# chalkydri/chalkydri

Measured on AMD Instinct MI355X. Metric: frames/sec (detect+pose) on 1280x800 batch; HBM GB/s vs roofline, higher is better.
Workload: dtype u8 (threshold/segment/clusters: integer; quad fit/decode/SQPnP: f64)

## Files before the change

chalkydri_amd/csrc/ck_internal.h:

```cpp
#ifndef CK_INTERNAL_H
#define CK_INTERNAL_H

#include <hip/hip_runtime.h>
#include <stdint.h>
#include <stdio.h>
#include <stdlib.h>

#include "chalkydri_hip.h"

typedef uint16_t ck_label_t;
#define CK_LBL_BORDER 0x8000u
#define CK_LBL_SMALL 0x4000u
#define CK_LBL_LOCAL_MASK 0x0FFFu
#define CK_LBL_ID_MASK 0x01FFu
#define CK_LBL_NONE 0xFFFFu
#define CK_LBL_INVALID 0xFFFFFFFFu

#define CK_TW 128
#define CK_TH 32
#define CK_RING_CAP (2 * (CK_TW + CK_TH))

__host__ __device__ inline uint32_t ck_label_slot(uint32_t l, int x, int y, int ccl_tiles_x) {
    return (uint32_t)((y / CK_TH) * ccl_tiles_x + x / CK_TW) * (uint32_t)CK_RING_CAP + (l & CK_LBL_ID_MASK);
}
__host__ __device__ inline uint32_t ck_label_interior_root(uint32_t l, int x, int y, int w) {
    return (uint32_t)((y & ~(CK_TH - 1)) + (int)((l >> 7) & (CK_TH - 1))) * (uint32_t)w + (uint32_t)((x & ~(CK_TW - 1)) + (int)(l & (CK_TW - 1)));
}

struct ck_border_root {
    uint32_t root;
    uint32_t size;
};

struct ck_dev_family {
    uint32_t nbits, ncodes, n_upstream;
    int32_t width_at_border, total_width, reversed_border;
    const uint64_t *codes;
    uint32_t bit_x[64], bit_y[64];
};

constexpr int CK_FIT_CLASSES = 8;
constexpr int CK_FIT_LISTS = 9;
constexpr int CK_EXT_PRE = 25, CK_EXT_POST = 24, CK_EXT_HALO = CK_EXT_PRE + CK_EXT_POST;
constexpr int CK_SPAN = 960;
constexpr int CK_HUGE_CAP = 65536, CK_HUGE_WGS = 256;
constexpr int CK_FIT_PARALLEL_MAX_FRAMES = 16;
constexpr int CK_SEG_CHUNKS_MAX = 8;
constexpr int CK_FIT_SIDE_STREAMS = 2;
constexpr int CK_LSCRATCH_PER_WG = 16384, CK_LSCRATCH_WGS = 1024;

typedef uint32_t ck_packed_point;
__host__ __device__ inline ck_cluster_point_t ck_unpack_point(ck_packed_point v) {
    const int k = (int)(v >> 1) & 3, sgn = (v & 1u) ? 1 : -1;
    const int dx = k == 2 ? -1 : (k == 1 ? 0 : 1), dy = k == 0 ? 0 : 1;
    ck_cluster_point_t p;
    p.x = (uint16_t)((v >> 16) & 0x1FFFu); p.y = (uint16_t)((v >> 3) & 0x1FFFu);
    p.gx = (int8_t)(dx * sgn); p.gy = (int8_t)(dy * sgn); p.pad = 0;
    return p;
}
struct ck_run {
    uint32_t slot;
    uint32_t base;
    uint32_t tmp_start;
    uint32_t count;
};

struct ck_stage_ws {
    int ht_size;
    int point_cap, cluster_cap, quad_cap, det_cap;
    int max_cluster_points;
    unsigned long long *d_ht_keys;
    uint32_t *d_ht_count;
    uint32_t *d_ht_off;
    ck_packed_point *d_tmp;
    ck_packed_point *d_points;
    int ext_cap;
    uint32_t *d_ext_xy;
    uint16_t *d_ext_w;
    double *d_maxval;
    uint16_t *d_maxpos;
    unsigned long long *d_maxmask;
    uint16_t *d_maxpre;
    long long *d_blk;
    uint32_t *d_cstate;
    ck_run *d_runs;
    int run_cap;
    unsigned long long *d_lscratch;
    unsigned long long *d_hscratch;
    int hcap;
    ck_cluster_t *d_clusters;
    uint32_t *d_counters;
    ck_quad_t *d_quads;
    ck_detection_t *d_dets;
    uint16_t *d_wimg;
    void *d_fit_scratch;
    size_t fit_scratch_bytes;
    ck_field_tag_t *d_field; int field_cap;
    double *d_gyro; uint8_t *d_has_gyro;
    ck_sqpnp_problem_t *d_problems;
    ck_iso3_t *d_pose_tags;
    double *d_bearings;
    double *d_world;
    ck_sqpnp_result_t *d_results;
    ck_vision_measurement_t *d_meas;
    int32_t *d_valid;
};
#define CK_CNT_TMP 0
#define CK_CNT_CLUSTERS 1
#define CK_CNT_POINTS 2
#define CK_CNT_QUADS 3
#define CK_CNT_DETS 4
#define CK_CNT_STATUS 5
#define CK_CNT_RUNS 6
#define CK_CNT_EXT 7
#define CK_CNT_STRIDE 8

struct ck_handle {
    ck_config_t cfg;
    int device;
    hipStream_t stream;
    hipStream_t stream2;
    hipEvent_t ev[16];
    hipEvent_t ev_fork, ev_join;
    hipStream_t fit_stream[CK_FIT_SIDE_STREAMS];
    hipStream_t seg_stream;
// ... 174 lines not shown
```

chalkydri_amd/csrc/k_quads.hip:

```cpp
#include <stdlib.h>

#include "ck_internal.h"

namespace {

struct FitArgs {
    const uint8_t *qim; int qw, qh, qstride; size_t qpitch;
    const uint16_t *wimg;
    const uint8_t *im; int w, h, stride; size_t pitch;
    int decimate, refine, max_nmaxima, min_tag_width, normal_ok, reversed_ok;
    double cos_critical, max_mse;
    ck_stage_ws ws;
    int stop_after;
    int guided;
    int list_cap;
    const uint32_t *list;
    const uint32_t *list_count;
    uint32_t *head;
};

struct M6 { long long Mx, My, Mxx, Mxy, Myy, W; };
__device__ __forceinline__ M6 m6_add(M6 a, M6 b) { a.Mx += b.Mx; a.My += b.My; a.Mxx += b.Mxx; a.Mxy += b.Mxy; a.Myy += b.Myy; a.W += b.W; return a; }
__device__ __forceinline__ M6 m6_sub(M6 a, M6 b) { a.Mx -= b.Mx; a.My -= b.My; a.Mxx -= b.Mxx; a.Mxy -= b.Mxy; a.Myy -= b.Myy; a.W -= b.W; return a; }
__device__ __forceinline__ M6 m6_zero() { M6 z = {0, 0, 0, 0, 0, 0}; return z; }
// ... 1231 lines not shown
#pragma unroll
                for (int e = 0; e < EPL; e++) {
                    const int i = tid + e * NTH;
                    if (i < sz0) {
                        const unsigned long long raw = stage(rawp[e]);
                        sKeys[i] = raw;
                        const int px = (int)(raw & 0xFFFF), py = (int)((raw >> 16) & 0xFFFF);
                        xmin = min(xmin, px); xmax = max(xmax, px);
                        ymin = min(ymin, py); ymax = max(ymax, py);
                    }
                }
            } else {
                for (int i = tid; i < sz0; i += NTH) {
                    const unsigned long long raw = stage(pts[i]);
                    sKeys[i] = raw;
                    const int px = (int)(raw & 0xFFFF), py = (int)((raw >> 16) & 0xFFFF);
                    xmin = min(xmin, px); xmax = max(xmax, px);
                    ymin = min(ymin, py); ymax = max(ymax, py);
                }
            }
            {
                int bb[4] = {xmin, -xmax, ymin, -ymax};
                B::reduce_min4(bb, iscr);
                xmin = bb[0]; xmax = -bb[1]; ymin = bb[2]; ymax = -bb[3];
            }
            if ((xmax - xmin) * (ymax - ymin) < a.min_tag_width) continue;
            if (a.stop_after == 10) continue;
            long long dot;
            {
                constexpr int EPLS = CAP / NTH;
                int n2 = NTH;
                while (n2 < sz0) n2 <<= 1;
                const int epl = n2 / NTH;
                B::sync();
                bool sorted = false;
                if constexpr (MLDS)
                    dot = keys_bucket_sort<NTH, EPLS>(sKeys, reinterpret_cast<uint32_t *>(sHist), sScratch, sz0, xmin, xmax, ymin, ymax,
                                                      a.normal_ok, a.reversed_ok, a.stop_after != 11, &sorted);
                else
                    dot = keys_bucket_sort_global<NTH, GK>(sKeys, reinterpret_cast<uint32_t *>(sHist), sScratch, scratch8, sz0, xmin, xmax, ymin, ymax,
                                                           a.normal_ok, a.reversed_ok, a.stop_after != 11, &sorted);
                if (sorted || GK) {}
                else if (EPLS >= 32 && epl == 32) dot = keys_sort<NTH, (EPLS >= 32 && !GK ? 32 : 1)>(sKeys, sScratch, sz0, xmin, xmax, ymin, ymax, a.normal_ok, a.reversed_ok, a.stop_after != 11);
                else if (EPLS >= 16 && epl == 16) dot = keys_sort<NTH, (EPLS >= 16 && !GK ? 16 : 1)>(sKeys, sScratch, sz0, xmin, xmax, ymin, ymax, a.normal_ok, a.reversed_ok, a.stop_after != 11);
                else if (EPLS >= 8 && epl == 8) dot = keys_sort<NTH, (EPLS >= 8 && !GK ? 8 : 1)>(sKeys, sScratch, sz0, xmin, xmax, ymin, ymax, a.normal_ok, a.reversed_ok, a.stop_after != 11);
                else if (EPLS >= 4 && epl == 4) dot = keys_sort<NTH, (EPLS >= 4 && !GK ? 4 : 1)>(sKeys, sScratch, sz0, xmin, xmax, ymin, ymax, a.normal_ok, a.reversed_ok, a.stop_after != 11);
                else if (EPLS >= 2 && epl == 2) dot = keys_sort<NTH, (EPLS >= 2 && !GK ? 2 : 1)>(sKeys, sScratch, sz0, xmin, xmax, ymin, ymax, a.normal_ok, a.reversed_ok, a.stop_after != 11);
                else dot = keys_sort<NTH, 1>(sKeys, sScratch, sz0, xmin, xmax, ymin, ymax, a.normal_ok, a.reversed_ok, a.stop_after != 11);
            }
            const int reversed = dot < 0;
            if (reversed && !a.reversed_ok) continue;
            if (!reversed && !a.normal_ok) continue;
            if (a.stop_after == 1 || a.stop_after == 11) continue;
            B::sync();
            int sz = 0;
            for (int base = 0; base < sz0; base += NTH) {
                const int i = base + tid;
                unsigned long long key = 0;
                int keep = 0;
                if (i < sz0) { key = sKeys[i]; keep = (i == 0) || (sKeys[i - 1] != key); }
                int tot = 0;
                const int incl = B::scan_flag(keep, iscr, &tot);
                B::sync();
                if (keep) sXY[sz + (int)incl - 1] = (uint32_t)(key & 0x3FFFFFFu);
                sz += (int)tot;
                B::sync();
            }
            if (sz < 24) continue;
            const int ksz = sz / 12 < 20 ? sz / 12 : 20;
            if (ksz < 2) continue;
            if (a.stop_after == 2) continue;
            if (tid == 0) sWork = atomicAdd(ws.d_counters + (size_t)frame * CK_CNT_STRIDE + CK_CNT_EXT, (uint32_t)(sz + CK_EXT_HALO));
            B::sync();
            const uint32_t es32 = sWork;
            uint32_t *exy = ws.d_ext_xy + (size_t)frame * ws.ext_cap + es32;
            for (int q = tid; q < sz + CK_EXT_HALO; q += NTH) {
                int src = q - CK_EXT_PRE;
                if (src < 0) src += sz;
                if (src < 0) src += sz;
                if (src >= sz) src -= sz;
                exy[q] = sXY[src] | ((uint32_t)ksz << 26);
            }
            if (tid == 0) { cstate[1] = es32; cstate[0] = (uint32_t)sz | (reversed ? 0x80000000u : 0u); }
        }
    }
}

constexpr int KL = 1024, KOFF = 32;
static_assert(CK_SPAN == 960 && KOFF >= CK_EXT_PRE + 3 && KL - KOFF - CK_SPAN >= CK_EXT_POST + 4, "span geometry");
__device__ __forceinline__ void k_chunk_body(const ck_stage_ws &ws, int qw, int qh) {
    __shared__ __attribute__((aligned(16))) unsigned long long sP64[3][KL];
    __shared__ __attribute__((aligned(16))) uint32_t sP32[3][KL];
    __shared__ uint8_t sKsz[KL];
    __shared__ unsigned long long sScan64[3][4];
    __shared__ uint32_t sScan32[3][4];
    __shared__ uint32_t sCnt[16];
    double *sS = reinterpret_cast<double *>(&sP64[0][0]), *sErr = reinterpret_cast<double *>(&sP64[1][0]);
    const int tid = threadIdx.x, lane = tid & 63, wv = tid >> 6;
    const int frame = blockIdx.y;
    const uint32_t *counters = ws.d_counters + (size_t)frame * CK_CNT_STRIDE;
    const uint32_t ext_total = min(counters[CK_CNT_EXT], (uint32_t)ws.ext_cap);
    const uint32_t *xy = ws.d_ext_xy + (size_t)frame * ws.ext_cap;
    uint16_t *w16 = ws.d_ext_w + (size_t)frame * ws.ext_cap;
    const uint16_t *wq = ws.d_wimg + (size_t)frame * qw * qh;
    double *mval = ws.d_maxval + (size_t)frame * (ws.ext_cap / 2);
    uint16_t *mpos = ws.d_maxpos + (size_t)frame * (ws.ext_cap / 2);
    unsigned long long *mmask = ws.d_maxmask + (size_t)frame * (ws.ext_cap / 64);
    uint16_t *mpre = ws.d_maxpre + (size_t)frame * (ws.ext_cap / 64);
    long long *blk = ws.d_blk + (size_t)frame * 6 * (ws.ext_cap / 32);
    auto load_xy = [&](uint32_t s) -> uint4 {
        const long long p0 = (long long)s * CK_SPAN - KOFF + 4 * tid;
        if ((unsigned long long)s * CK_SPAN < ext_total && p0 >= 0 && p0 + 4 <= (long long)ws.ext_cap) return *reinterpret_cast<const uint4 *>(xy + p0);
        return make_uint4(0, 0, 0, 0);
    };
    auto gather_w = [&](uint32_t v) -> uint32_t {
        const int x = (int)((v >> 13) & 0x1FFFu), y = (int)(v & 0x1FFFu);
        const int ix = (x + 1) >> 1, iy = (y + 1) >> 1;
        return (ix < qw && iy < qh) ? (uint32_t)wq[(size_t)iy * qw + ix] : 1u;
    };
    uint4 x4 = load_xy(blockIdx.x);
    uint32_t ww[4] = {gather_w(x4.x), gather_w(x4.y), gather_w(x4.z), gather_w(x4.w)};
    for (uint32_t s = blockIdx.x; (unsigned long long)s * CK_SPAN < ext_total; s += gridDim.x) {
        __builtin_amdgcn_s_waitcnt(WAIT_VMCNT0);
        const long long p0 = (long long)s * CK_SPAN - KOFF + 4 * tid;
        const uint32_t xw[4] = {x4.x, x4.y, x4.z, x4.w};
        if (tid >= KOFF / 4 && tid < (KOFF + CK_SPAN) / 4)
            *reinterpret_cast<uint2 *>(w16 + p0) = make_uint2(ww[0] | (ww[1] << 16), ww[2] | (ww[3] << 16));
        unsigned long long l64[4][3];
        uint32_t l32[4][3];
        unsigned long long a64[3] = {0, 0, 0};
        uint32_t a32[3] = {0, 0, 0};
#pragma unroll
        for (int e = 0; e < 4; e++) {
            const M6 m = moments_of(xw[e] & 0x3FFFFFFu, ww[e]);
            a64[0] += (unsigned long long)m.Mxx; a64[1] += (unsigned long long)m.Mxy; a64[2] += (unsigned long long)m.Myy;
            a32[0] += (uint32_t)m.Mx; a32[1] += (uint32_t)m.My; a32[2] += (uint32_t)m.W;
#pragma unroll
            for (int q = 0; q < 3; q++) { l64[e][q] = a64[q]; l32[e][q] = a32[q]; }
        }
        unsigned long long x64[3];
        uint32_t x32[3];
#pragma unroll
        for (int q = 0; q < 3; q++) { x64[q] = wave_scan_u64(a64[q]); x32[q] = wave_scan_u32(a32[q]); }
        lds_barrier();
        if (lane == 63)
#pragma unroll
            for (int q = 0; q < 3; q++) { sScan64[q][wv] = x64[q]; sScan32[q][wv] = x32[q]; }
        lds_barrier();
#pragma unroll
        for (int q = 0; q < 3; q++) {
            unsigned long long b64 = 0;
            uint32_t b32 = 0;
            for (int k = 0; k < wv; k++) { b64 += sScan64[q][k]; b32 += sScan32[q][k]; }
            x64[q] += b64 - a64[q]; x32[q] += b32 - a32[q];
        }
#pragma unroll
        for (int e = 0; e < 4; e++) {
            const int j = 4 * tid + e;
#pragma unroll
            for (int q = 0; q < 3; q++) { sP64[q][j] = l64[e][q] + x64[q]; sP32[q][j] = l32[e][q] + x32[q]; }
            const uint32_t k = (xw[e] >> 26) & 31u;
            sKsz[j] = (uint8_t)(k > 20u ? 20u : k);
        }
        const uint4 nx4 = load_xy(s + gridDim.x);
        lds_barrier();
        if (tid < 180) {
// ... 651 lines not shown
                double dp = f01.nx * f12.nx + f01.ny * f12.ny;
                if (fabs(dp) > a.cos_critical) continue;
                const PairFit f23 = sF[m2 * MAXSEL + m3];
                if (f23.mse > a.max_mse) continue;
                const PairFit f30 = sF[m3 * MAXSEL + m0];
                if (f30.mse > a.max_mse) continue;
                double e = f01.err + f12.err + f23.err + f30.err;
                if (e < best || (e == best && pk < bestc)) { best = e; bestc = pk; }
            }
        }
#pragma unroll
        for (int d = 32; d >= 1; d >>= 1) {
            double ob = __shfl_xor(best, d, 64);
            int oc = __shfl_xor(bestc, d, 64);
            if (ob < best || (ob == best && oc < bestc)) { best = ob; bestc = oc; }
        }
        if (best == HUGE_VAL) continue;
        FDBG(4);
        if (best / (double)sz >= a.max_mse) continue;
        FDBG(5);

        if (a.stop_after == 7) continue;
        if (tid < 4) {
            const int sel[4] = {(bestc >> 12) & 15, (bestc >> 8) & 15, (bestc >> 4) & 15, bestc & 15};
            int N;
            const int s0 = sel[tid], s1 = sel[(tid + 1) & 3];
            const M6 m = rangeM(s0, s1, &N);
            const PairFit pf = sF[s0 * MAXSEL + s1];
            SideRec r;
            r.Mx = m.Mx; r.My = m.My; r.W = m.W; r.nx = pf.nx; r.ny = pf.ny; r.mse = pf.mse;
            sB[nb][tid] = r;
        }
        if (tid == 0) { sBMeta[nb][0] = (uint32_t)frame; sBMeta[nb][1] = (uint32_t)reversed; sBMeta[nb][2] = rep0; sBMeta[nb][3] = rep1; }
        nb++;
        wave_sync();
        if (nb == BATCH) flush();
        }
        if (nb) flush();
    }
}

__global__ __launch_bounds__(64) __attribute__((amdgpu_waves_per_eu(4, 8))) void k_tail(FitArgs a) { k_tail_body(a); }

__global__ __launch_bounds__(256) void k_weight_image(const uint8_t *__restrict__ qim, size_t qpitch, int qstride, int qw, int qh,
                                                      uint16_t *__restrict__ wimg) {
    const int w4 = (qw + 3) >> 2;
    const int g = blockIdx.x * 64 + (threadIdx.x & 63), iy = blockIdx.y * 4 + (threadIdx.x >> 6);
    if (g >= w4 || iy >= qh) return;
    const size_t fr = blockIdx.z;
    const int ix = 4 * g;
    uint16_t out[4] = {1, 1, 1, 1};
    if (iy > 0 && iy + 1 < qh) {
        const uint8_t *row = qim + fr * qpitch + (size_t)iy * qstride + ix;
        const uint32_t mid = *reinterpret_cast<const uint32_t *>(row);
        const uint32_t up = *reinterpret_cast<const uint32_t *>(row - qstride), dn = *reinterpret_cast<const uint32_t *>(row + qstride);
        const int left = ix > 0 ? (int)row[-1] : 0, right = ix + 4 < qw ? (int)row[4] : 0;
        const int m[6] = {left, (int)(mid & 255u), (int)((mid >> 8) & 255u), (int)((mid >> 16) & 255u), (int)(mid >> 24), right};
#pragma unroll
        for (int k = 0; k < 4; k++) {
            const int x = ix + k;
            if (x > 0 && x + 1 < qw) {
                const int gx = m[k + 2] - m[k];
                const int gy = (int)((dn >> (8 * k)) & 255u) - (int)((up >> (8 * k)) & 255u);
                out[k] = (uint16_t)(isqrt_u32((uint32_t)(gx * gx + gy * gy)) + 1);
            }
        }
    }
    uint16_t *dst = wimg + fr * ((size_t)qw * qh) + (size_t)iy * qw + ix;
    if ((qw & 3) == 0)
        *reinterpret_cast<uint2 *>(dst) = make_uint2((uint32_t)out[0] | ((uint32_t)out[1] << 16), (uint32_t)out[2] | ((uint32_t)out[3] << 16));
    else {
#pragma unroll
        for (int k = 0; k < 4; k++)
            if (ix + k < qw) dst[k] = out[k];
    }
}

__global__ __launch_bounds__(1024) void k_classify(ck_stage_ws ws, int n, uint32_t *lists, uint32_t *list_counts, int list_cap, int split) {
    __shared__ uint32_t sCnt[CK_FIT_LISTS], sBase[CK_FIT_LISTS];
    const int frame = blockIdx.x, tid = threadIdx.x;
    const uint32_t *counters = ws.d_counters + (size_t)frame * CK_CNT_STRIDE;
    const uint32_t nc = counters[CK_CNT_CLUSTERS];
    const ck_cluster_t *cls = ws.d_clusters + (size_t)frame * ws.cluster_cap;
    auto class_of = [split](uint32_t c) { return (c <= 256 && (split & 2)) ? 7 : c <= 512 ? 0 : (c <= 1024 && (split & 1)) ? 6 : (c <= 2048 ? 1 : (c <= 4096 ? 2 : (c <= 8192 ? 3 : (c <= 16384 ? 4 : 5)))); };
    if (tid < CK_FIT_LISTS) sCnt[tid] = 0;
    __syncthreads();
    for (uint32_t i = tid; i < nc; i += 1024) if (cls[i].count) { atomicAdd(&sCnt[class_of(cls[i].count)], 1u); atomicAdd(&sCnt[CK_FIT_CLASSES], 1u); }
    __syncthreads();
    if (tid < CK_FIT_LISTS) { sBase[tid] = sCnt[tid] ? atomicAdd(&list_counts[tid], sCnt[tid]) : 0u; }
    __syncthreads();
    if (tid < CK_FIT_LISTS) sCnt[tid] = 0;
    __syncthreads();
    for (uint32_t i = tid; i < nc; i += 1024) {
        if (!cls[i].count) continue;
        const int k = class_of(cls[i].count);
        const uint32_t pos = sBase[k] + atomicAdd(&sCnt[k], 1u);
        if (pos < (uint32_t)list_cap) lists[(size_t)k * list_cap + pos] = ((uint32_t)frame << 20) | i;
        const uint32_t pa = sBase[CK_FIT_CLASSES] + atomicAdd(&sCnt[CK_FIT_CLASSES], 1u);
        if (pa < (uint32_t)list_cap) lists[(size_t)CK_FIT_CLASSES * list_cap + pa] = ((uint32_t)frame << 20) | i;
    }
}
}

#ifdef CK_FLAT_DEBUG
extern "C" int ck_flat_debug_read(unsigned int *out, int reset) {
    unsigned int z[32] = {};
    if (hipMemcpyFromSymbol(out, HIP_SYMBOL(g_flat_dbg), sizeof z) != hipSuccess) return -1;
    if (reset && hipMemcpyToSymbol(HIP_SYMBOL(g_flat_dbg), z, sizeof z) != hipSuccess) return -1;
    return 0;
}
#endif
#ifdef CK_FIT_PROFILE
extern "C" int ck_fit_profile_read(unsigned long long *out, int reset) {
    unsigned long long z[3][16] = {};
    if (hipMemcpyFromSymbol(out, HIP_SYMBOL(g_fit_prof), sizeof z) != hipSuccess) return -1;
    if (reset && hipMemcpyToSymbol(HIP_SYMBOL(g_fit_prof), z, sizeof z) != hipSuccess) return -1;
    return 0;
}
#endif

int ck_launch_fit_quads(ck_handle *h, const ck_dev_image &qimg, const ck_dev_image &img, int n) {
    ck_stage_ws &ws = h->ws;
    if (n > 4095 || ws.cluster_cap > (1 << 20)) return CK_EINVAL;
    const ck_fit_layout fl = ck_fit_scratch_layout(ws, h->cfg.max_batch);
    const int list_cap = fl.list_cap;
    uint32_t *lists = fl.lists, *list_counts = fl.list_counts, *heads = fl.heads;
    static const int fit_split = CK_KNOB("CK_FIT_SPLIT", 3);
    static const int force_par = CK_KNOB("CK_FIT_PAR", 0);
    const bool side_by_side = n <= (h->cfg.quad_decimate > 1 ? 2 * CK_FIT_PARALLEL_MAX_FRAMES : CK_FIT_PARALLEL_MAX_FRAMES) || force_par;
    const int split = side_by_side ? 0 : fit_split;
    hipLaunchKernelGGL(k_classify, dim3((unsigned)n), dim3(1024), 0, h->stream, ws, n, lists, list_counts, list_cap, split);
    FitArgs a;
    a.qim = qimg.p; a.qw = h->qw; a.qh = h->qh; a.qstride = qimg.stride; a.qpitch = qimg.pitch;
    a.wimg = ws.d_wimg;
    auto launch_wimg = [&](hipStream_t st) {
        const int w4 = (h->qw + 3) / 4;
        hipLaunchKernelGGL(k_weight_image, dim3((unsigned)((w4 + 63) / 64), (unsigned)((h->qh + 3) / 4), (unsigned)n), dim3(256), 0, st, qimg.p,
                           qimg.pitch, qimg.stride, h->qw, h->qh, ws.d_wimg);
    };
    static const int flat_env0 = CK_KNOB("CK_FIT_FLAT", 1);
    static const int wimg_aside_env = CK_KNOB("CK_FIT_WIMG_ASIDE", 1);
    static const int tails_aside_ok0 = CK_KNOB("CK_FIT_TAILS_ASIDE", 1) && ck_streams_wanted() < 2;
    const bool flat0 = flat_env0 >= 2 || (flat_env0 == 1 && !side_by_side && (size_t)n * (size_t)h->qw * (size_t)h->qh >= ((size_t)100 << 20));
    const bool wimg_aside = flat0 && !side_by_side && tails_aside_ok0 && wimg_aside_env;
    if (!wimg_aside) launch_wimg(h->stream);
    a.im = img.p; a.w = h->w; a.h = h->h; a.stride = img.stride; a.pitch = img.pitch;
    a.decimate = h->cfg.quad_decimate; a.refine = h->cfg.refine_edges; a.max_nmaxima = h->cfg.max_nmaxima;
    a.cos_critical = h->cfg.cos_critical_rad; a.max_mse = h->cfg.max_line_fit_mse;
    a.normal_ok = 0; a.reversed_ok = 0; a.min_tag_width = 1 << 30;
    for (int f = 0; f < h->cfg.n_families; f++) {
        const ck_family_t *fam = h->cfg.families[f];
        if (fam->width_at_border < a.min_tag_width) a.min_tag_width = fam->width_at_border;
        if (fam->reversed_border) a.reversed_ok = 1; else a.normal_ok = 1;
    }
    a.min_tag_width /= h->cfg.quad_decimate;
    if (a.min_tag_width < 3) a.min_tag_width = 3;
    a.ws = ws; a.list_cap = list_cap;
    a.stop_after = CK_KNOB("CK_FIT_STOP_AFTER", 99);
    a.guided = CK_KNOB("CK_FIT_GUIDED", 1);
    int cus = 256;
    hipStream_t cs[CK_FIT_CLASSES] = {h->stream, h->stream, h->stream, h->stream, h->stream, h->stream, h->stream, h->stream};
    static const int tails_aside_ok = tails_aside_ok0;
    const bool tails_aside = !side_by_side && tails_aside_ok;
    if (side_by_side) { cs[3] = h->fit_stream[0]; cs[2] = h->fit_stream[1]; cs[4] = h->fit_stream[1]; }
    if (tails_aside) { cs[4] = h->fit_stream[0]; cs[5] = h->fit_stream[0]; cs[3] = h->fit_stream[0]; }
    static const int aside_env = CK_KNOB0("CK_FIT_ASIDE", -1);
    if (tails_aside && aside_env >= 0)
        for (int c = 0; c < CK_FIT_CLASSES; c++) cs[c] = ((aside_env >> c) & 1) ? h->fit_stream[0] : (((aside_env >> (8 + c)) & 1) ? h->fit_stream[1] : h->stream);
    if (side_by_side || tails_aside) {
        CK_HIP(hipEventRecord(h->ev_fit_fork, h->stream));
        for (int k = 0; k < CK_FIT_SIDE_STREAMS; k++) CK_HIP(hipStreamWaitEvent(h->fit_stream[k], h->ev_fit_fork, 0));
        if (wimg_aside) launch_wimg(h->fit_stream[1]);
    }
    static const int gk_env = CK_KNOB("CK_FIT_GK", 0);
    const int gk_mask = ws.d_hscratch && !side_by_side ? gk_env : 0;
    static const int skip_mask = CK_KNOB("CK_FIT_SKIP", 0);
    static const int flat_env = flat_env0;
    const bool flat = flat_env >= 2 || (flat_env == 1 && !side_by_side && (size_t)n * (size_t)h->qw * (size_t)h->qh >= ((size_t)100 << 20));
    static const int seq_alt = CK_KNOB("CK_SEQ_ALT", 0);
    static const int seq_wgs0 = CK_KNOB("CK_SEQ_WGS0", 16), seq_wgs7 = CK_KNOB("CK_SEQ_WGS7", 16), seq_wgs6 = CK_KNOB("CK_SEQ_WGS6", 8);
    auto launch_split = [&](int c) {
        switch (c) {
        case 0: hipLaunchKernelGGL((k_seq<64, 512, true, 4, false>), dim3((unsigned)(cus * seq_wgs0)), dim3(64), 0, cs[c], a); break;
        case 7: hipLaunchKernelGGL((k_seq<64, 256, true, 4, false>), dim3((unsigned)(cus * seq_wgs7)), dim3(64), 0, cs[c], a); break;
        case 6: hipLaunchKernelGGL((k_seq<128, 1024, true, 4, false>), dim3((unsigned)(cus * seq_wgs6)), dim3(128), 0, cs[c], a); break;
        case 1: hipLaunchKernelGGL((k_seq<256, 2048, true, 4, false>), dim3((unsigned)(cus * 4)), dim3(256), 0, cs[c], a); break;
        case 2: if (seq_alt & 16) hipLaunchKernelGGL((k_seq<256, 4096, true, 2, false>), dim3((unsigned)(cus * 2)), dim3(256), 0, cs[c], a);
                else hipLaunchKernelGGL((k_seq<256, 4096, true, 3, false>), dim3((unsigned)(cus * 3)), dim3(256), 0, cs[c], a);
                break;
        case 3: hipLaunchKernelGGL((k_seq<512, 8192, true, 2, false>), dim3((unsigned)cus), dim3(512), 0, cs[c], a); break;
        case 4: hipLaunchKernelGGL((k_seq<512, 16384, false, 2, false>), dim3((unsigned)cus), dim3(512), 0, cs[c], a); break;
        default:
            if (ws.d_hscratch) hipLaunchKernelGGL((k_seq<512, CK_HUGE_CAP, false, 2, true>), dim3((unsigned)CK_HUGE_WGS), dim3(512), 0, cs[c], a);
            break;
        }
    };
    auto launch = [&](int c) {
        if ((skip_mask >> c) & 1) return;
        a.list = lists + (size_t)c * list_cap; a.list_count = list_counts + c; a.head = heads + c;
        if (flat) { launch_split(c); return; }
        switch (c) {
        case 0: { static const int s_wgs = CK_KNOB("CK_FIT_S_WGS", 12);
            hipLaunchKernelGGL((k_fit<64, 512, 64, true, 3>), dim3((unsigned)(cus * s_wgs)), dim3(64), 0, cs[c], a); break; }
        case 7: hipLaunchKernelGGL((k_fit<64, 256, 64, true, 4>), dim3((unsigned)(cus * 16)), dim3(64), 0, cs[c], a); break;
        case 6: hipLaunchKernelGGL((k_fit<128, 1024, 128, true, 4>), dim3((unsigned)(cus * 7)), dim3(128), 0, cs[c], a); break;
        case 1: hipLaunchKernelGGL((k_fit<256, 2048, 224, true, 4>), dim3((unsigned)(cus * 4)), dim3(256), 0, cs[c], a); break;
        case 2: hipLaunchKernelGGL((k_fit<256, 4096, 512, true, 2>), dim3((unsigned)(cus * 2)), dim3(256), 0, cs[c], a); break;
        case 3:
            if (gk_mask & 8) hipLaunchKernelGGL((k_fit<512, 16384, 512, false, 4, true>), dim3((unsigned)CK_HUGE_WGS), dim3(512), 0, cs[c], a);
            else hipLaunchKernelGGL((k_fit<512, 8192, 896, true, 2>), dim3((unsigned)cus), dim3(512), 0, cs[c], a);
            break;
        case 4:
            if (gk_mask & 16) hipLaunchKernelGGL((k_fit<512, 16384, 512, false, 4, true>), dim3((unsigned)CK_HUGE_WGS), dim3(512), 0, cs[c], a);
            else hipLaunchKernelGGL((k_fit<512, 16384, 512, false, 2>), dim3((unsigned)cus), dim3(512), 0, cs[c], a);
            break;
        default:
            if (ws.d_hscratch) hipLaunchKernelGGL((k_fit<512, CK_HUGE_CAP, 896, false, 2, true>), dim3((unsigned)CK_HUGE_WGS), dim3(512), 0, cs[c], a);
            break;
        }
    };
    if (side_by_side) { launch(3); launch(2); launch(4); launch(0); launch(1); launch(5); }
    else if (tails_aside) { launch(4); launch(5); launch(3); launch(7); launch(0); launch(6); launch(1); launch(2); }
    else { launch(7); launch(0); launch(6); for (int c = 1; c < 6; c++) launch(c); }
    if (side_by_side || tails_aside)
        for (int k = 0; k < CK_FIT_SIDE_STREAMS; k++) {
            CK_HIP(hipEventRecord(h->ev_fit_join[k], h->fit_stream[k]));
            CK_HIP(hipStreamWaitEvent(h->stream, h->ev_fit_join[k], 0));
        }
    if (flat) {
        const unsigned spans = (unsigned)(ws.ext_cap / CK_SPAN);
        static const int chunk_wgs = CK_KNOB("CK_CHUNK_WGS", 64);
        static const int tail_wgs = CK_KNOB("CK_TAIL_WGS", 16);
        unsigned gx = (unsigned)((cus * chunk_wgs + n - 1) / n);
        if (gx < 8) gx = 8;
        if (gx > spans) gx = spans;
        if (a.stop_after > 3) hipLaunchKernelGGL(k_chunk, dim3(gx, (unsigned)n), dim3(256), 0, h->stream, ws, h->qw, h->qh);
        a.list = lists + (size_t)CK_FIT_CLASSES * list_cap; a.list_count = list_counts + CK_FIT_CLASSES; a.head = heads + CK_FIT_CLASSES;
        hipLaunchKernelGGL(k_tail, dim3((unsigned)(cus * tail_wgs)), dim3(64), 0, h->stream, a);
    }
    CK_HIP(hipGetLastError());
    return CK_OK;
}
```

Before: 17940.

## Add paired half-wave kernel for tiny clusters in flat fit path

Adds a new size class for clusters of at most 128 points and a k_seq_pair kernel that handles two clusters per 64-lane wave, one per 32-lane half. It uses DPP half-wave reductions and scans, plus a shared-memory bucket sort with a rank fix-up. The goal is to avoid wasting half a wave, and the per-cluster sync overhead, on small clusters that k_seq<64,256> processed one at a time. The class is only enabled in the flat (large-batch) path by default. It adds another kernel launch and a more complex sort whose correctness must match the existing one.

```diff
diff --git a/chalkydri_amd/csrc/ck_internal.h b/chalkydri_amd/csrc/ck_internal.h
--- a/chalkydri_amd/csrc/ck_internal.h
+++ b/chalkydri_amd/csrc/ck_internal.h
@@ -39,8 +39,8 @@
     uint32_t bit_x[64], bit_y[64];
 };
 
-constexpr int CK_FIT_CLASSES = 8;
-constexpr int CK_FIT_LISTS = 9;
+constexpr int CK_FIT_CLASSES = 9;
+constexpr int CK_FIT_LISTS = 10;
 constexpr int CK_EXT_PRE = 25, CK_EXT_POST = 24, CK_EXT_HALO = CK_EXT_PRE + CK_EXT_POST;
 constexpr int CK_SPAN = 960;
 constexpr int CK_HUGE_CAP = 65536, CK_HUGE_WGS = 256;
diff --git a/chalkydri_amd/csrc/k_quads.hip b/chalkydri_amd/csrc/k_quads.hip
--- a/chalkydri_amd/csrc/k_quads.hip
+++ b/chalkydri_amd/csrc/k_quads.hip
@@ -1337,6 +1337,234 @@
                 exy[q] = sXY[src] | ((uint32_t)ksz << 26);
             }
             if (tid == 0) { cstate[1] = es32; cstate[0] = (uint32_t)sz | (reversed ? 0x80000000u : 0u); }
+        }
+    }
+}
+
+__device__ __forceinline__ int half_min_i32(int x) {
+    x = min(x, __builtin_amdgcn_update_dpp(x, x, 0x111, 0xF, 0xF, false));
+    x = min(x, __builtin_amdgcn_update_dpp(x, x, 0x112, 0xF, 0xF, false));
+    x = min(x, __builtin_amdgcn_update_dpp(x, x, 0x114, 0xF, 0xF, false));
+    x = min(x, __builtin_amdgcn_update_dpp(x, x, 0x118, 0xF, 0xF, false));
+    x = min(x, __builtin_amdgcn_update_dpp(x, x, 0x142, 0xA, 0xF, false));
+    const int lo = __builtin_amdgcn_readlane(x, 31), hi = __builtin_amdgcn_readlane(x, 63);
+    return (threadIdx.x & 32) ? hi : lo;
+}
+__device__ __forceinline__ uint32_t half_scan_u32(uint32_t x) {
+    x += dpp0<0x111, 0xF>(x); x += dpp0<0x112, 0xF>(x); x += dpp0<0x114, 0xF>(x); x += dpp0<0x118, 0xF>(x);
+    x += dpp0<0x142, 0xA>(x);
+    return x;
+}
+__device__ __forceinline__ long long half_sum_i64(long long v) {
+    unsigned long long x = (unsigned long long)v;
+    x += dpp0_64<0x111, 0xF>(x); x += dpp0_64<0x112, 0xF>(x); x += dpp0_64<0x114, 0xF>(x); x += dpp0_64<0x118, 0xF>(x);
+    x += dpp0_64<0x142, 0xA>(x);
+    const uint32_t l0 = (uint32_t)__builtin_amdgcn_readlane((int)(uint32_t)x, 31), l1 = (uint32_t)__builtin_amdgcn_readlane((int)(x >> 32), 31);
+    const uint32_t h0 = (uint32_t)__builtin_amdgcn_readlane((int)(uint32_t)x, 63), h1 = (uint32_t)__builtin_amdgcn_readlane((int)(x >> 32), 63);
+    return (long long)((threadIdx.x & 32) ? ((unsigned long long)h1 << 32) | h0 : ((unsigned long long)l1 << 32) | l0);
+}
+
+template <int EPL>
+__global__ __launch_bounds__(64) __attribute__((amdgpu_waves_per_eu(4, 8))) void k_seq_pair(FitArgs a) {
+    constexpr int CAPH = 32 * EPL;
+    constexpr int NB = CAPH, PER = NB / 32;
+    constexpr int LGQ = (NB == 256 ? 8 : (NB == 128 ? 7 : 6)) - 3;
+    static_assert(NB == 64 || NB == 128 || NB == 256, "bucket count");
+    __shared__ unsigned long long sKeys2[2][CAPH];
+    __shared__ uint32_t sHist2[2][NB + 1];
+    __shared__ uint32_t sWork;
+    __shared__ uint32_t sHItem[64], sHStart[64], sHCount[64];
+    const int tid = threadIdx.x, half = tid >> 5, hl = tid & 31;
+    const ck_stage_ws &ws = a.ws;
+    unsigned long long *const sKeys = sKeys2[half];
+    uint32_t *const hist = sHist2[half];
+    uint32_t *const sXY = reinterpret_cast<uint32_t *>(sKeys);
+    const uint32_t n_work = min(*a.list_count, (uint32_t)a.list_cap);
+    constexpr uint32_t DQMAX = 64u;
+    const uint32_t per_wg4 = (n_work / (gridDim.x * 4u)) & ~1u;
+    const uint32_t DQ = per_wg4 < 2u ? 2u : (per_wg4 > DQMAX ? DQMAX : per_wg4);
+    const uint32_t static_total = gridDim.x * DQ;
+    uint32_t chunk_base = blockIdx.x * DQ, chunk_len = DQ, dq_next = DQ;
+    bool first_chunk = true;
+    auto stage = [](ck_packed_point v) -> unsigned long long {
+        const int k = (int)(v >> 1) & 3, sgn = (v & 1u) ? 1 : -1;
+        const int dx = k == 2 ? -1 : (k == 1 ? 0 : 1), dy = k == 0 ? 0 : 1;
+        return (unsigned long long)((v >> 16) & 0x1FFFu) | ((unsigned long long)((v >> 3) & 0x1FFFu) << 16) |
+               ((unsigned long long)(uint8_t)(int8_t)(dx * sgn) << 32) | ((unsigned long long)(uint8_t)(int8_t)(dy * sgn) << 40);
+    };
+    for (;;) {
+        if (!first_chunk) {
+            if (static_total >= n_work) break;
+            wave_sync();
+            if (tid == 0) sWork = static_total + atomicAdd(a.head, dq_next);
+            wave_sync();
+            chunk_base = sWork;
+            chunk_len = dq_next;
+            if (a.guided) {
+                const uint32_t g = chunk_base < n_work ? ((n_work - chunk_base) / (gridDim.x * 2u)) & ~1u : 0u;
+                dq_next = g < 2u ? 2u : (g > DQ ? DQ : g);
+            }
+        }
+        first_chunk = false;
+        if (chunk_base >= n_work) break;
+        const int len = (int)min(chunk_len, n_work - chunk_base);
+        wave_sync();
+        if (tid < len) {
+            const uint32_t item = a.list[chunk_base + (uint32_t)tid];
+            const ck_cluster_t cl = ws.d_clusters[(size_t)(item >> 20) * ws.cluster_cap + (item & 0xFFFFFu)];
+            sHItem[tid] = item; sHStart[tid] = cl.start; sHCount[tid] = cl.count;
+        }
+        wave_sync();
+        ck_packed_point nxt[EPL];
+        auto fetch = [&](int k) {
+            const int kk = k + half;
+            const bool have = kk < len;
+            const uint32_t item = have ? sHItem[kk] : 0u, cnt = have ? sHCount[kk] : 0u;
+            const ck_packed_point *p = ws.d_points + (size_t)(item >> 20) * ws.ext_cap + (have ? sHStart[kk] : 0u);
+#pragma unroll
+            for (int e = 0; e < EPL; e++) { const uint32_t i = (uint32_t)(hl + e * 32); nxt[e] = (i < cnt && cnt <= (uint32_t)CAPH) ? p[i] : 0u; }
+        };
+        fetch(0);
+        for (int k = 0; k < len; k += 2) {
+            const int kk = k + half;
+            const bool have = kk < len;
+            const uint32_t item = have ? sHItem[kk] : 0u;
+            const int frame = (int)(item >> 20), ci = (int)(item & 0xFFFFFu);
+            const int sz0 = have ? (int)sHCount[kk] : 0;
+            ck_packed_point rawp[EPL];
+            __builtin_amdgcn_s_waitcnt(WAIT_VMCNT0);
+#pragma unroll
+            for (int e = 0; e < EPL; e++) rawp[e] = nxt[e];
+            if (k + 2 < len) fetch(k + 2);
+            wave_sync();
+            uint32_t *cstate = ws.d_cstate + 2 * ((size_t)frame * ws.cluster_cap + ci);
+            if (hl == 0 && have) *cstate = 0u;
+            int n0 = (have && sz0 >= 1 && sz0 <= CAPH && a.stop_after != 0) ? sz0 : 0;
+            int xmin = 1 << 30, xmax = -(1 << 30), ymin = 1 << 30, ymax = -(1 << 30);
+#pragma unroll
+            for (int e = 0; e < EPL; e++) {
+                const int i = hl + e * 32;
+                if (i < n0) {
+                    const unsigned long long raw = stage(rawp[e]);
+                    const int px = (int)(raw & 0xFFFF), py = (int)((raw >> 16) & 0xFFFF);
+                    xmin = min(xmin, px); xmax = max(xmax, px);
+                    ymin = min(ymin, py); ymax = max(ymax, py);
+                }
+            }
+            xmin = half_min_i32(xmin); xmax = -half_min_i32(-xmax); ymin = half_min_i32(ymin); ymax = -half_min_i32(-ymax);
+            if (n0 && (xmax - xmin) * (ymax - ymin) < a.min_tag_width) n0 = 0;
+            if (a.stop_after == 10) n0 = 0;
+            for (int i = hl; i <= NB; i += 32) hist[i] = 0;
+            unsigned long long kreg[EPL];
+            uint32_t meta[EPL];
+            long long dot = 0;
+#pragma unroll
+            for (int e = 0; e < EPL; e++) {
+                const int i = hl + e * 32;
+                kreg[e] = 0; meta[e] = 0;
+                if (i < n0) {
+                    const unsigned long long raw = stage(rawp[e]);
+                    const int px = (int)(raw & 0xFFFF), py = (int)((raw >> 16) & 0xFFFF);
+                    const int pgx = (int)(signed char)((raw >> 32) & 0xFF), pgy = (int)(signed char)((raw >> 40) & 0xFF);
+                    const int dx = 4 * px - 2 * (xmin + xmax) - 1, dy = 4 * py - 2 * (ymin + ymax) + 1;
+                    dot += (long long)(dx * pgx + dy * pgy);
+                    kreg[e] = angle_key(px, py, xmin, xmax, ymin, ymax);
+                }
+            }
+            dot = half_sum_i64(dot);
+            const int reversed = dot < 0;
+            if (reversed ? !a.reversed_ok : !a.normal_ok) n0 = 0;
+            if (a.stop_after == 11) n0 = 0;
+            if (__ballot(n0 != 0) == 0ull) continue;
+            wave_sync();
+#pragma unroll
+            for (int e = 0; e < EPL; e++) {
+                const int i = hl + e * 32;
+                if (i < n0) {
+                    const uint32_t oct = (uint32_t)(kreg[e] >> 57), frac = (uint32_t)(kreg[e] >> 26) & 0x7FFFFFFFu;
+                    uint32_t fb = frac >> (30 - LGQ);
+                    fb = fb > (1u << LGQ) - 1 ? (1u << LGQ) - 1 : fb;
+                    const uint32_t b = (oct << LGQ) | fb;
+                    meta[e] = (b << 16) | atomicAdd(&hist[b], 1u);
+                }
+            }
+            wave_sync();
+            {
+                uint32_t c[PER], sum = 0;
+#pragma unroll
+                for (int q = 0; q < PER; q++) { c[q] = hist[hl * PER + q]; sum += c[q]; }
+                uint32_t run = half_scan_u32(sum) - sum;
+#pragma unroll
+                for (int q = 0; q < PER; q++) { hist[hl * PER + q] = run; run += c[q]; }
+                if (hl == 31) hist[NB] = run;
+            }
+            wave_sync();
+#pragma unroll
+            for (int e = 0; e < EPL; e++) {
+                const int i = hl + e * 32;
+                if (i < n0) sKeys[hist[meta[e] >> 16] + (meta[e] & 0xFFFFu)] = kreg[e];
+            }
+            wave_sync();
+            uint32_t pos[EPL];
+#pragma unroll
+            for (int e = 0; e < EPL; e++) {
+                const int i = hl + e * 32;
+                pos[e] = 0;
+                if (i < n0) {
+                    const uint32_t b = meta[e] >> 16, s0 = hist[b], s1 = hist[b + 1], mine = s0 + (meta[e] & 0xFFFFu);
+                    const unsigned long long key = kreg[e];
+                    uint32_t rank = 0;
+                    for (uint32_t j = s0; j < s1; j++) {
+                        const unsigned long long o = sKeys[j];
+                        rank += (o < key || (o == key && j < mine)) ? 1u : 0u;
+                    }
+                    pos[e] = s0 + rank;
+                }
+            }
+            wave_sync();
+#pragma unroll
+            for (int e = 0; e < EPL; e++) {
+                const int i = hl + e * 32;
+                if (i < n0) sKeys[pos[e]] = kreg[e];
+            }
+            if (a.stop_after == 1) n0 = 0;
+            wave_sync();
+            int sz = 0;
+            const int nmax = max(__builtin_amdgcn_readlane(n0, 0), __builtin_amdgcn_readlane(n0, 32));
+            for (int base = 0; base < nmax; base += 32) {
+                const int i = base + hl;
+                unsigned long long key = 0;
+                int keep = 0;
+                if (i < n0) { key = sKeys[i]; keep = (i == 0) || (sKeys[i - 1] != key); }
+                const unsigned long long bal = __ballot(keep != 0);
+                const uint32_t mine = half ? (uint32_t)(bal >> 32) : (uint32_t)bal;
+                const int incl = __popc(mine & ((2u << hl) - 1u));
+                wave_sync();
+                if (keep) sXY[sz + incl - 1] = (uint32_t)(key & 0x3FFFFFFu);
+                sz += __popc(mine);
+                wave_sync();
+            }
+            if (sz < 24) n0 = 0;
+            const int ksz = sz / 12 < 20 ? sz / 12 : 20;
+            if (ksz < 2) n0 = 0;
+            if (a.stop_after == 2) n0 = 0;
+            uint32_t es32 = 0;
+            if (hl == 0 && n0) es32 = atomicAdd(ws.d_counters + (size_t)frame * CK_CNT_STRIDE + CK_CNT_EXT, (uint32_t)(sz + CK_EXT_HALO));
+            {
+                const uint32_t lo = (uint32_t)__builtin_amdgcn_readlane((int)es32, 0), hi = (uint32_t)__builtin_amdgcn_readlane((int)es32, 32);
+                es32 = half ? hi : lo;
+            }
+            if (n0) {
+                uint32_t *exy = ws.d_ext_xy + (size_t)frame * ws.ext_cap + es32;
+                for (int q = hl; q < sz + CK_EXT_HALO; q += 32) {
+                    int src = q - CK_EXT_PRE;
+                    if (src < 0) src += sz;
+                    if (src < 0) src += sz;
+                    if (src >= sz) src -= sz;
+                    exy[q] = sXY[src] | ((uint32_t)ksz << 26);
+                }
+                if (hl == 0) { cstate[1] = es32; cstate[0] = (uint32_t)sz | (reversed ? 0x80000000u : 0u); }
+            }
         }
     }
 }
@@ -2154,7 +2382,7 @@
     const uint32_t *counters = ws.d_counters + (size_t)frame * CK_CNT_STRIDE;
     const uint32_t nc = counters[CK_CNT_CLUSTERS];
     const ck_cluster_t *cls = ws.d_clusters + (size_t)frame * ws.cluster_cap;
-    auto class_of = [split](uint32_t c) { return (c <= 256 && (split & 2)) ? 7 : c <= 512 ? 0 : (c <= 1024 && (split & 1)) ? 6 : (c <= 2048 ? 1 : (c <= 4096 ? 2 : (c <= 8192 ? 3 : (c <= 16384 ? 4 : 5)))); };
+    auto class_of = [split](uint32_t c) { return (c <= 128 && (split & 4)) ? 8 : (c <= 256 && (split & 2)) ? 7 : c <= 512 ? 0 : (c <= 1024 && (split & 1)) ? 6 : (c <= 2048 ? 1 : (c <= 4096 ? 2 : (c <= 8192 ? 3 : (c <= 16384 ? 4 : 5)))); };
     if (tid < CK_FIT_LISTS) sCnt[tid] = 0;
     __syncthreads();
     for (uint32_t i = tid; i < nc; i += 1024) if (cls[i].count) { atomicAdd(&sCnt[class_of(cls[i].count)], 1u); atomicAdd(&sCnt[CK_FIT_CLASSES], 1u); }
@@ -2200,7 +2428,10 @@
     static const int fit_split = CK_KNOB("CK_FIT_SPLIT", 3);
     static const int force_par = CK_KNOB("CK_FIT_PAR", 0);
     const bool side_by_side = n <= (h->cfg.quad_decimate > 1 ? 2 * CK_FIT_PARALLEL_MAX_FRAMES : CK_FIT_PARALLEL_MAX_FRAMES) || force_par;
-    const int split = side_by_side ? 0 : fit_split;
+    static const int flat_env0 = CK_KNOB("CK_FIT_FLAT", 1);
+    const bool flat0 = flat_env0 >= 2 || (flat_env0 == 1 && !side_by_side && (size_t)n * (size_t)h->qw * (size_t)h->qh >= ((size_t)100 << 20));
+    static const int fit_pair = CK_KNOB("CK_FIT_PAIR", 2);
+    const int split = (side_by_side ? 0 : fit_split) | (flat0 && (fit_pair & 2) ? 4 : 0);
     hipLaunchKernelGGL(k_classify, dim3((unsigned)n), dim3(1024), 0, h->stream, ws, n, lists, list_counts, list_cap, split);
     FitArgs a;
     a.qim = qimg.p; a.qw = h->qw; a.qh = h->qh; a.qstride = qimg.stride; a.qpitch = qimg.pitch;
@@ -2210,10 +2441,8 @@
         hipLaunchKernelGGL(k_weight_image, dim3((unsigned)((w4 + 63) / 64), (unsigned)((h->qh + 3) / 4), (unsigned)n), dim3(256), 0, st, qimg.p,
                            qimg.pitch, qimg.stride, h->qw, h->qh, ws.d_wimg);
     };
-    static const int flat_env0 = CK_KNOB("CK_FIT_FLAT", 1);
     static const int wimg_aside_env = CK_KNOB("CK_FIT_WIMG_ASIDE", 1);
     static const int tails_aside_ok0 = CK_KNOB("CK_FIT_TAILS_ASIDE", 1) && ck_streams_wanted() < 2;
-    const bool flat0 = flat_env0 >= 2 || (flat_env0 == 1 && !side_by_side && (size_t)n * (size_t)h->qw * (size_t)h->qh >= ((size_t)100 << 20));
     const bool wimg_aside = flat0 && !side_by_side && tails_aside_ok0 && wimg_aside_env;
     if (!wimg_aside) launch_wimg(h->stream);
     a.im = img.p; a.w = h->w; a.h = h->h; a.stride = img.stride; a.pitch = img.pitch;
@@ -2231,14 +2460,14 @@
     a.stop_after = CK_KNOB("CK_FIT_STOP_AFTER", 99);
     a.guided = CK_KNOB("CK_FIT_GUIDED", 1);
     int cus = 256;
-    hipStream_t cs[CK_FIT_CLASSES] = {h->stream, h->stream, h->stream, h->stream, h->stream, h->stream, h->stream, h->stream};
+    hipStream_t cs[CK_FIT_CLASSES] = {h->stream, h->stream, h->stream, h->stream, h->stream, h->stream, h->stream, h->stream, h->stream};
     static const int tails_aside_ok = tails_aside_ok0;
     const bool tails_aside = !side_by_side && tails_aside_ok;
     if (side_by_side) { cs[3] = h->fit_stream[0]; cs[2] = h->fit_stream[1]; cs[4] = h->fit_stream[1]; }
     if (tails_aside) { cs[4] = h->fit_stream[0]; cs[5] = h->fit_stream[0]; cs[3] = h->fit_stream[0]; }
     static const int aside_env = CK_KNOB0("CK_FIT_ASIDE", -1);
     if (tails_aside && aside_env >= 0)
-        for (int c = 0; c < CK_FIT_CLASSES; c++) cs[c] = ((aside_env >> c) & 1) ? h->fit_stream[0] : (((aside_env >> (8 + c)) & 1) ? h->fit_stream[1] : h->stream);
+        for (int c = 0; c < 8; c++) cs[c] = ((aside_env >> c) & 1) ? h->fit_stream[0] : (((aside_env >> (8 + c)) & 1) ? h->fit_stream[1] : h->stream);
     if (side_by_side || tails_aside) {
         CK_HIP(hipEventRecord(h->ev_fit_fork, h->stream));
         for (int k = 0; k < CK_FIT_SIDE_STREAMS; k++) CK_HIP(hipStreamWaitEvent(h->fit_stream[k], h->ev_fit_fork, 0));
@@ -2251,10 +2480,12 @@
     const bool flat = flat_env >= 2 || (flat_env == 1 && !side_by_side && (size_t)n * (size_t)h->qw * (size_t)h->qh >= ((size_t)100 << 20));
     static const int seq_alt = CK_KNOB("CK_SEQ_ALT", 0);
     static const int seq_wgs0 = CK_KNOB("CK_SEQ_WGS0", 16), seq_wgs7 = CK_KNOB("CK_SEQ_WGS7", 16), seq_wgs6 = CK_KNOB("CK_SEQ_WGS6", 8);
+    static const int seq_wgs8 = CK_KNOB("CK_SEQ_WGS8", 16);
     auto launch_split = [&](int c) {
         switch (c) {
         case 0: hipLaunchKernelGGL((k_seq<64, 512, true, 4, false>), dim3((unsigned)(cus * seq_wgs0)), dim3(64), 0, cs[c], a); break;
         case 7: hipLaunchKernelGGL((k_seq<64, 256, true, 4, false>), dim3((unsigned)(cus * seq_wgs7)), dim3(64), 0, cs[c], a); break;
+        case 8: hipLaunchKernelGGL((k_seq_pair<4>), dim3((unsigned)(cus * seq_wgs8)), dim3(64), 0, cs[c], a); break;
         case 6: hipLaunchKernelGGL((k_seq<128, 1024, true, 4, false>), dim3((unsigned)(cus * seq_wgs6)), dim3(128), 0, cs[c], a); break;
         case 1: hipLaunchKernelGGL((k_seq<256, 2048, true, 4, false>), dim3((unsigned)(cus * 4)), dim3(256), 0, cs[c], a); break;
         case 2: if (seq_alt & 16) hipLaunchKernelGGL((k_seq<256, 4096, true, 2, false>), dim3((unsigned)(cus * 2)), dim3(256), 0, cs[c], a);
@@ -2271,6 +2502,7 @@
         if ((skip_mask >> c) & 1) return;
         a.list = lists + (size_t)c * list_cap; a.list_count = list_counts + c; a.head = heads + c;
         if (flat) { launch_split(c); return; }
+        if (c == 8) return;
         switch (c) {
         case 0: { static const int s_wgs = CK_KNOB("CK_FIT_S_WGS", 12);
             hipLaunchKernelGGL((k_fit<64, 512, 64, true, 3>), dim3((unsigned)(cus * s_wgs)), dim3(64), 0, cs[c], a); break; }
@@ -2291,9 +2523,9 @@
             break;
         }
     };
-    if (side_by_side) { launch(3); launch(2); launch(4); launch(0); launch(1); launch(5); }
-    else if (tails_aside) { launch(4); launch(5); launch(3); launch(7); launch(0); launch(6); launch(1); launch(2); }
-    else { launch(7); launch(0); launch(6); for (int c = 1; c < 6; c++) launch(c); }
+    if (side_by_side) { launch(3); launch(2); launch(4); launch(8); launch(0); launch(1); launch(5); }
+    else if (tails_aside) { launch(4); launch(5); launch(3); launch(8); launch(7); launch(0); launch(6); launch(1); launch(2); }
+    else { launch(8); launch(7); launch(0); launch(6); for (int c = 1; c < 6; c++) launch(c); }
     if (side_by_side || tails_aside)
         for (int k = 0; k < CK_FIT_SIDE_STREAMS; k++) {
             CK_HIP(hipEventRecord(h->ev_fit_join[k], h->fit_stream[k]));
```

Result: no change. 17930 (-0.1%).
